# KAIST-VICLab/pronerf

Hardware: AMD Instinct MI355X
Metric: rays/sec (and ms/1008x756 frame) LLFF Fern 8-sample infer (higher is better)
Workload: dtype bf16 (NeRF MLP operands) + f16 (refine MLP operands); fp32 accumulate + f16 | f16x2 (sampler MLP: plain fp16 pass for every ray, split fp16 hi+lo operands = fp32-grade for the rays whose depth order that pass cannot decide; fp32 accumulate)

## Files before the change

include/pronerf_hip.h:

```cpp
#ifndef PRONERF_HIP_H
#define PRONERF_HIP_H

#include <stdint.h>

#ifdef __cplusplus
extern "C" {
#endif

#define PNRF_ABI_VERSION 1

#define PNRF_E_ARG (-1)
#define PNRF_E_SHAPE (-2)
#define PNRF_E_STATE (-3)

#define PNRF_NET_SAMPLER 0
#define PNRF_NET_REFINE 1
#define PNRF_NET_NERF 2
#define PNRF_NET_NERFCLS 3

typedef struct pnrf_mlp pnrf_mlp_t;
typedef struct pnrf_ctx pnrf_ctx_t;
typedef struct pnrf_trainer pnrf_trainer_t;
typedef struct pnrf_scene pnrf_scene_t;

// ... 54 lines not shown
                          float* refine_in, int64_t n, void* stream);
int pnrf_refine_input_train_fwd(const float* rays, const float* or_rays, const float* depth_sorted,
                                const float* img4, const float* poses, const float* K, const int64_t* ref_nos,
                                int nv, int nb, int Hf, int Wf, float eps, int layout, float* refine_in,
                                int64_t n, void* stream);
int pnrf_composite_fwd(const float* raw, const float* z, const float* rays_d, int d_stride,
                       const float* add, const float* mul, const float* noise, float clamp,
                       int white_bkgd, float* rgb, float* disp, float* acc, float* weights,
                       float* depth, int64_t n, int s, void* stream);

int pnrf_sampler_fwd(const pnrf_mlp_t* h, const float* rays, int64_t n, float* depth_sorted,
                     float* add_sorted, float* mul_sorted, int64_t* sort_idx, float* mm_rgb,
                     float* depth_raw, void* stream);
#define PNRF_SAMPLER_KAPPA 2.0f
int64_t pnrf_sampler_workspace_bytes(int64_t n);
int pnrf_sampler_fwd_ws(const pnrf_mlp_t* h, const float* rays, int64_t n, float* depth_sorted, float* add_sorted,
                        float* mul_sorted, int64_t* sort_idx, float* mm_rgb, float* depth_raw, void* workspace,
                        int64_t workspace_bytes, float kappa, void* stream);
int pnrf_refine_fwd(const pnrf_mlp_t* h, const float* refine_in, const float* rays,
                    const float* depth_sorted, float* z, float* pts, int64_t n, void* stream);
int pnrf_refine_project_fwd(const pnrf_mlp_t* h, const float* rays, const float* or_rays, const float* depth_sorted,
                            const float* img4, const float* proj, int nb, int Hf, int Wf, float eps, float* z,
                            float* pts, int64_t n, void* stream);
int pnrf_refine_train_fwd(const pnrf_mlp_t* h, const float* refine_in, const float* rays,
                          const float* depth_sorted, const float* jitter, int jitter_dir, float* z, float* pts,
                          float* rgb0, int64_t n, void* stream);
int pnrf_nerf_fwd(const pnrf_mlp_t* h, const float* pts, const float* rays, const float* z,
                  const float* add_sorted, const float* mul_sorted, float* rgbd, float* raw,
                  int64_t n, void* stream);

int pnrf_nerf_train_fwd(const pnrf_mlp_t* h, const float* pts, const float* rays, const float* z,
                        const float* add_sorted, const float* mul_sorted, const float* noise, float clamp,
                        int white_bkgd, int S, float* rgbd, float* raw, int64_t n, void* stream);
int pnrf_explore_fwd(const float* z8, const float* rays, const float* jitter, int n_mult, int dir1, int dir2,
                     float* z_out, float* pts_out, int64_t n, void* stream);

int pnrf_ctx_create(const pnrf_mlp_t* sampler, const pnrf_mlp_t* refine, const pnrf_mlp_t* nerf,
                    int64_t max_rays, pnrf_ctx_t** out);
int pnrf_ctx_free(pnrf_ctx_t* ctx);
int pnrf_render_rays_fwd(pnrf_ctx_t* ctx, const float* rays, const float* or_rays,
                         const float* img4, const float* proj, int nb, int Hf, int Wf, float eps,
                         float* rgbd, int64_t* sort_idx, int64_t n, void* stream);
int pnrf_ctx_set_sampler_kappa(pnrf_ctx_t* ctx, float kappa);
int pnrf_ctx_get_sampler_kappa(const pnrf_ctx_t* ctx, float* kappa);
int pnrf_ctx_sampler_stats(pnrf_ctx_t* ctx, int64_t* rays_second_pass);
int pnrf_ctx_sampler_saturated(pnrf_ctx_t* ctx, int64_t* rays_third_pass);
#define PNRF_NERF_SKIP_NEVER 0
#define PNRF_NERF_SKIP_AUTO 1
#define PNRF_NERF_SKIP_ALWAYS 2
#define PNRF_NERF_SKIP_MIN_RAYS 8192
#define PNRF_NERF_SKIP_DEAD_PERCENT 2
int pnrf_ctx_set_nerf_skip(pnrf_ctx_t* ctx, int mode);
int pnrf_ctx_nerf_live(pnrf_ctx_t* ctx, int64_t* live_columns, int* list_mode);
int pnrf_ctx_profile_begin(pnrf_ctx_t* ctx, int max_frames);
int pnrf_ctx_profile_end(pnrf_ctx_t* ctx, float* ms, int* frames);


int pnrf_composite_bwd(const float* raw, const float* z, const float* rays_d, int d_stride, const float* add,
                       const float* mul, const float* noise, float clamp, int white_bkgd, const float* d_rgb,
                       float* d_raw, float* d_z, float* d_add, float* d_mul, int64_t n, int s, void* stream);
int pnrf_composite_bwd_maps(const float* raw, const float* z, const float* rays_d, int d_stride, const float* add,
                            const float* mul, const float* noise, float clamp, int white_bkgd, const float* d_rgb,
                            const float* d_disp, const float* d_acc, const float* d_weights, const float* d_depth,
                            const float* d_z_in, float* d_raw, float* d_z, float* d_add, float* d_mul, int64_t n, int s,
                            void* stream);
int pnrf_posenc_bwd(const float* x, const float* d_out, float* d_x, int64_t n, int n_freq, void* stream);
// ... 134 lines not shown
```

pronerf_amd/_lib.py:

```python
from __future__ import annotations

import ctypes as C
import os

_HERE = os.path.dirname(os.path.abspath(__file__))
LIB_PATH = os.path.join(_HERE, 'lib', 'libpronerf_hip.so')

NET_SAMPLER, NET_REFINE, NET_NERF, NET_NERFCLS = 0, 1, 2, 3
VARIANTS = {'default': 0, 'sampler_f32': 1, 'sampler_f32_full': 2, 'bf16_32x32': 3, 'nerf_4x64': 4, 'sampler_split': 5, 'bf16': 6, 'f16': 7, 'refine_16x16': 8}
ABI_VERSION = 1


class PnrfError(RuntimeError):
    pass


_p = C.c_void_p
_i64 = C.c_int64
_f = C.c_float
_i = C.c_int

SIGNATURES = {
    'pnrf_abi_version': (_i, []),
    'pnrf_last_error': (C.c_char_p, []),
    'pnrf_mlp_pack': (_i, [_i, C.POINTER(_p), C.POINTER(_p), C.POINTER(_i), C.POINTER(_i), _i, C.POINTER(_p)]),
    'pnrf_mlp_pack_image': (_i, [_i, C.POINTER(_p), C.POINTER(_p), C.POINTER(_i), C.POINTER(_i), _i, _p, _i64, C.POINTER(_i64)]),
    'pnrf_mlp_repack': (_i, [_p, C.POINTER(_p), C.POINTER(_p), C.POINTER(_i), C.POINTER(_i), _i, _p]),
    'pnrf_mlp_free': (_i, [_p]),
    'pnrf_mlp_serialize': (_i, [_p, _p, _i64, C.POINTER(_i64)]),
    'pnrf_mlp_deserialize': (_i, [_p, _i64, C.POINTER(_p)]),
    'pnrf_mlp_kind': (_i, [_p, C.POINTER(_i), C.POINTER(_i), C.POINTER(_i), C.POINTER(_i)]),
    'pnrf_mlp_skips': (_i, [_p, C.POINTER(C.c_uint32)]),
    'pnrf_mlp_set_variant': (_i, [_p, _i]),
    'pnrf_mlp_set_shape': (_i, [_p, _i]),
    'pnrf_mlp_fwd': (_i, [_p, _p, _p, _p, _i64, _i, _p]),
    'pnrf_posenc_fwd': (_i, [_p, _p, _i64, _i, _p]),
    'pnrf_plucker_fwd': (_i, [_p, _p, _p, _i64, _p]),
    'pnrf_ray_encode_fwd': (_i, [_p, _p, _i64, _i, _p]),
    'pnrf_frame_rays_fwd': (_i, [C.POINTER(_f), C.POINTER(_f), _i, _i, _f, _f, _f, _f, _i64, _i64, _p, _p, _p]),
    'pnrf_frame_rays_blocks_fwd': (_i, [C.POINTER(_f), C.POINTER(_f), _i, _i, _f, _f, _f, _f, _i64, _i64, _i64, _i64, _p, _p, _p]),
    'pnrf_ndc_rays_fwd': (_i, [_p, _p, _i, _i, _f, _f, _p, _p, _i64, _p]),
    'pnrf_warp_trt_fwd': (_i, [_p, _p, _p, _p, _i64, _p, _p, _i, _i, _i, _i64, _p]),
    'pnrf_warp_train_fwd': (_i, [_p, _p, _p, _p, _i64, _p, _p, _p, _i, _i, _i, _i64, _p]),
    'pnrf_refine_input_train_fwd': (_i, [_p, _p, _p, _p, _p, _p, _p, _i, _i, _i, _i, _f, _i, _p, _i64, _p]),
    'pnrf_refine_train_fwd': (_i, [_p, _p, _p, _p, _p, _i, _p, _p, _p, _i64, _p]),
    'pnrf_nerf_train_fwd': (_i, [_p, _p, _p, _p, _p, _p, _p, _f, _i, _i, _p, _p, _i64, _p]),
    'pnrf_explore_fwd': (_i, [_p, _p, _p, _i, _i, _i, _p, _p, _i64, _p]),
    'pnrf_images_pack': (_i, [_p, _p, _i, _i, _i, _p]),
    'pnrf_refine_input_fwd': (_i, [_p, _p, _p, _p, _p, _i, _i, _i, _f, _p, _i64, _p]),
    'pnrf_composite_fwd': (_i, [_p, _p, _p, _i, _p, _p, _p, _f, _i, _p, _p, _p, _p, _p, _i64, _i, _p]),
    'pnrf_sampler_fwd': (_i, [_p, _p, _i64, _p, _p, _p, _p, _p, _p, _p]),
    'pnrf_sampler_workspace_bytes': (_i64, [_i64]),
    'pnrf_sampler_fwd_ws': (_i, [_p, _p, _i64, _p, _p, _p, _p, _p, _p, _p, _i64, _f, _p]),
    'pnrf_refine_fwd': (_i, [_p, _p, _p, _p, _p, _p, _i64, _p]),
    'pnrf_refine_project_fwd': (_i, [_p, _p, _p, _p, _p, _p, _i, _i, _i, _f, _p, _p, _i64, _p]),
    'pnrf_nerf_fwd': (_i, [_p, _p, _p, _p, _p, _p, _p, _p, _i64, _p]),
    'pnrf_ctx_create': (_i, [_p, _p, _p, _i64, C.POINTER(_p)]),
    'pnrf_ctx_free': (_i, [_p]),
    'pnrf_render_rays_fwd': (_i, [_p, _p, _p, _p, _p, _i, _i, _i, _f, _p, _p, _i64, _p]),
    'pnrf_ctx_sampler_stats': (_i, [_p, C.POINTER(_i64)]),
    'pnrf_ctx_set_sampler_kappa': (_i, [_p, _f]),
    'pnrf_ctx_get_sampler_kappa': (_i, [_p, C.POINTER(_f)]),
    'pnrf_ctx_sampler_saturated': (_i, [_p, C.POINTER(_i64)]),
    'pnrf_ctx_set_nerf_skip': (_i, [_p, _i]),
    'pnrf_ctx_nerf_live': (_i, [_p, C.POINTER(_i64), C.POINTER(_i)]),
    'pnrf_ctx_profile_begin': (_i, [_p, _i]),
    'pnrf_ctx_profile_end': (_i, [_p, C.POINTER(C.c_float), C.POINTER(_i)]),
    'pnrf_linspace': (_i, [_f, _f, _i, C.POINTER(_f)]),
    'pnrf_image_metrics_workspace_bytes': (_i64, [_i, _i, _i]),
    'pnrf_image_metrics_fwd': (_i, [_p, _i, _p, _i, _i, _i, C.POINTER(_f), _i, _f, _f, _f, _p, _p, _p, _i64, _p]),
    'pnrf_ssim_loss_workspace_bytes': (_i64, [_i, _i, _i, _i]),
    'pnrf_ssim_loss_fwd': (_i, [_p, _i, _i64, _p, _i, _i64, _i, _i, _i, C.POINTER(_f), _i, _f, _f, _f, _p, _p, _p, _i64, _p]),
    'pnrf_frame_to8b_fwd': (_i, [_p, _i, _p, _i, _i64, _p, _p, _p, _i64, _p]),
    'pnrf_png_segment_rows': (_i, []),
    'pnrf_png_max_bytes': (_i64, [_i, _i, _i]),
    'pnrf_png_workspace_bytes': (_i64, [_i, _i, _i]),
    'pnrf_png_encode_host': (_i, [_p, _i64, _i, _i, _i, _i, _p, _i64, C.POINTER(_i64)]),
    'pnrf_png_encode_fwd': (_i, [_p, _i64, _i, _i, _i, _i, _p, _i64, _p, _p, _i64, _p]),
    'pnrf_lpips_create': (_i, [C.c_char_p, C.POINTER(_p), C.POINTER(_p), C.POINTER(_i), _i, C.POINTER(_p), C.POINTER(_i), C.POINTER(_p)]),
    'pnrf_lpips_free': (_i, [_p]),
    'pnrf_lpips_tap_dims': (_i, [C.c_char_p, _i, _i, C.POINTER(_i)]),
    'pnrf_lpips_workspace_bytes': (_i64, [_p, _i, _i]),
    'pnrf_lpips_fwd': (_i, [_p, _p, _i, _p, _i, _i, _i, _i, _p, _p, _p, _i64, _p]),
    'pnrf_lpips_layer_workspace_bytes': (_i64, [_p, _i, _i, _i, _i]),
    'pnrf_lpips_layer_fwd': (_i, [_p, _i, _i, _p, _i, _i, _p, _p, _i64, _p]),
    'pnrf_lpips_loss_workspace_bytes': (_i64, [_p, _i, _i, _i]),
    'pnrf_lpips_loss_fwd': (_i, [_p, _p, _i, _i64, _p, _i, _i64, _i, _i, _i, _i, _p, _p, _p, _i64, _p]),
    'pnrf_lpips_layer_bwd_workspace_bytes': (_i64, [_p, _i, _i, _i, _i, _i]),
    'pnrf_lpips_layer_bwd': (_i, [_p, _i, _i, _i, _i, _p, _i, _i, _p, _p, _p, _p, _i64, _p]),
# ... 89 lines not shown
```

pronerf_amd/csrc/pnrf_mlp_kernels.hip:

```cpp
#include <type_traits>

#include "pnrf_common.h"
#include "pnrf_geom.h"

#ifndef PNRF_LAST_TMAX
#define PNRF_LAST_TMAX 1
#endif
#ifndef PNRF_OLD_PRIO
#define PNRF_OLD_PRIO 0
#endif
#ifndef PNRF_YOUNG_PRIO
#define PNRF_YOUNG_PRIO 1
#endif

using namespace pnrf;

namespace {



template <int N, int I = 0, class F>
__device__ __forceinline__ void static_for(F&& f) {
  if constexpr (I < N) {
    f(std::integral_constant<int, I>{});
// ... 1675 lines not shown
  }
  return make_float4(s0, s1, s2, s3);
}

typedef __bf16 bf16x2_t __attribute__((ext_vector_type(2)));
__device__ __forceinline__ int relu_pack_bf16(float a, float b) {
#ifdef PNRF_RELU_F32
  return __builtin_bit_cast(int, bf16x2_t{(__bf16)act_fast(a, ACT_RELU), (__bf16)act_fast(b, ACT_RELU)});
#else
  int pk;
  asm("v_cvt_pk_bf16_f32 %0, %1, %2" : "=v"(pk) : "v"(a), "v"(b));
  return __builtin_bit_cast(int, __builtin_elementwise_max(__builtin_bit_cast(i16x2_t, pk), i16x2_t{0, 0}));
#endif
}
template <class P>
__device__ __forceinline__ int relu_pack(float a, float b) {
  if constexpr (std::is_same<P, PrecBf16>::value) return relu_pack_bf16(a, b);
  return __builtin_bit_cast(int, __builtin_elementwise_max(__builtin_bit_cast(i16x2_t, P::cvt_pk(a, b)), i16x2_t{0, 0}));
}
template <int NCB, class P = PrecBf16>
struct HiddenEpi16 {
  typename P::v8 (&Bn)[NCB][NB_KS_H];
  __device__ __forceinline__ void operator()(int tp, int pc, f32x4 (&acc)[2][NCB], int cb0) const {
#pragma unroll
    for (int cb = cb0; cb < cb0 + 2; ++cb) {
      i32x4_t w = __builtin_bit_cast(i32x4_t, Bn[cb][tp]);
      w[2 * pc] = relu_pack<P>(acc[pc][cb][0], acc[pc][cb][1]);
      w[2 * pc + 1] = relu_pack<P>(acc[pc][cb][2], acc[pc][cb][3]);
      Bn[cb][tp] = __builtin_bit_cast(typename P::v8, w);
    }
  }
};

template <bool CLS, int NCB, class P, int NW, bool LIST>
__device__ __forceinline__ void nerf16_body(const NerfArgs& a) {
  constexpr int TPB = 64 * NW;
  using Epi = HiddenEpi16<NCB, P>;
  using v8 = typename P::v8;
  if (a.skip && a.skip[SKIP_MODE] != (LIST ? SKIP_MODE_LIST : SKIP_MODE_DENSE)) return;
  const int nlive = LIST ? a.skip[SKIP_LIVE] : 0;
  const int nbatch = LIST ? (nlive + NW * 16 * NCB - 1) / (NW * 16 * NCB) : a.nbatch;
  if constexpr (LIST) {
    if ((int)blockIdx.x >= nbatch) {
      if (threadIdx.x == 0 && atomicAdd(a.queue + 1, 1) == (int)gridDim.x - 1) { a.queue[0] = 0; a.queue[1] = 0; }
      return;
    }
  }
  P::enter();
  extern __shared__ __attribute__((aligned(16))) char smem[];
  float* bias_lds = (float*)(smem + RING_BYTES);
  WStream<NW> st;
  st.init(a.blob, a.nslots, smem);
  st.prologue();
  for (int i = threadIdx.x; i < a.nbias; i += TPB) bias_lds[i] = a.bias[i];
  __syncthreads();
  const int lane = threadIdx.x & 63, wave = threadIdx.x >> 6, c16 = lane & 15, g = lane >> 4;
  int pe_c[4];
  float pe_sc[4];
#pragma unroll
  for (int j4 = 0; j4 < 4; ++j4) {
    const int q = 4 * g + j4;
    pe_c[j4] = q % 3;
    pe_sc[j4] = (float)(1 << (2 * (q / 3)));
  }
  const float pe_vs = (float)(1 << g);
  const int64_t nrows = a.n * a.S;
  own_the_simd<NW>();
  young_half_priority<NW>();
  const char* ringlane = smem + lane * 16;
  const float* biaslane = bias_lds + 4 * g;
  const bool composite = !LIST && a.S == 8 && a.rgbd;

  __shared__ __attribute__((aligned(16))) int s_next[4];
  for (int batch = blockIdx.x; batch < nbatch;) {
    int q_pend = 0;
    if (a.queue && threadIdx.x == 0) q_pend = atomicAdd(a.queue, 1);
    int64_t row[NCB];
    bool valid[NCB];
    v8 Bo[NCB][NB_KS_H], Bn[NCB][NB_KS_H], Bx[NCB];
    float e_dn[NCB], e_z[NCB], e_add[NCB], e_mul[NCB], e_noise[NCB];
    static_for<NCB>([&](auto cbc) {
      constexpr int cb = decltype(cbc)::value;
      row[cb] = (int64_t)batch * (NW * 16 * NCB) + wave * (16 * NCB) + cb * 16 + c16;
      valid[cb] = row[cb] < (LIST ? (int64_t)nlive : nrows);
      int64_t rr = valid[cb] ? row[cb] : nrows - 1;
      if constexpr (LIST) {
        rr = a.list[valid[cb] ? row[cb] : (int64_t)nlive - 1];
        row[cb] = rr;
      }
      const float* pp = a.pts + rr * 3;
      const float* ry = a.rays + (a.S == 8 ? (rr >> 3) : rr / a.S) * 11;
      const float x3[3] = {pp[0], pp[1], pp[2]};
      const float v3[3] = {ry[8], ry[9], ry[10]};
      if (composite) {
        e_dn[cb] = ray_dir_norm(ry);
        e_z[cb] = a.z[rr]; e_add[cb] = a.add ? a.add[rr] : 0.f; e_mul[cb] = a.mul ? a.mul[rr] : 1.f;
        e_noise[cb] = a.noise ? a.noise[rr] : 0.f;
      }
      float f0[16], fx[8];
#pragma unroll
      for (int j4 = 0; j4 < 4; ++j4) {
        const float xv = pe_c[j4] == 0 ? x3[0] : (pe_c[j4] == 1 ? x3[1] : x3[2]);
        float s, co;
        pe_sincos_scaled(xv, pe_sc[j4], s, co);
        f0[4 * j4 + 0] = s; f0[4 * j4 + 1] = co;
        f0[4 * j4 + 2] = 2.f * s * co; f0[4 * j4 + 3] = (co - s) * (co + s);
      }
      if (g == 3) { f0[12] = x3[0]; f0[13] = x3[1]; f0[14] = x3[2]; f0[15] = 0.f; }
#pragma unroll
      for (int c = 0; c < 3; ++c) pe_sincos_scaled(v3[c], pe_vs, fx[2 * c], fx[2 * c + 1]);
      fx[6] = g == 0 ? v3[0] : (g == 1 ? v3[2] : 0.f);
      fx[7] = g == 0 ? v3[1] : 0.f;
#pragma unroll
      for (int ks = 0; ks < NB_KS0; ++ks) {
        float v[8];
#pragma unroll
        for (int j = 0; j < 8; ++j) v[j] = f0[ks * 8 + j];
        Bo[cb][ks] = P::pack(v);
      }
      Bx[cb] = P::pack(fx);
    });
    f32x4 fin[2][NCB], pend[2][NCB];
    if constexpr (!CLS) {
      auto hidden = [&](v8(&in)[NCB][NB_KS_H], v8(&out)[NCB][NB_KS_H], int l) {
        f32x4 np[2][NCB];
        layer_b16<NB_KS_H, NB_NTP_H, NB_POS_H, NCB, v8>(st, ringlane, biaslane + (1 + l) * W_HID, [&](int cb, int ks) { return in[cb][ks]; }, Epi{out},
                                               [&](int pc, int cb0) { Epi{in}(NB_NTP_H - 1, pc, pend, cb0); }, np);
#pragma unroll
        for (int t = 0; t < 2; ++t)
#pragma unroll
          for (int cb = 0; cb < NCB; ++cb) pend[t][cb] = np[t][cb];
      };
      layer_b16<NB_KS0, NB_NTP_H, 0, NCB, v8>(st, ringlane, biaslane, [&](int cb, int ks) { return Bo[cb][ks < NB_KS0 ? ks : 0]; }, Epi{Bn}, [](int, int) {}, pend);
      const int nhid = PNRF_NHID(a.nhid, N_NHID);
      auto last_layer = [&](v8(&in)[NCB][NB_KS_H]) {
        layer_b16<NB_KS_LAST, 1, NB_POS_LAST, NCB, v8, PNRF_LAST_TMAX>(
            st, ringlane, biaslane + (1 + nhid) * W_HID, [&](int cb, int ks) { return ks < NB_KS_H ? in[cb][ks < NB_KS_H ? ks : 0] : Bx[cb]; },
            [&](int, int, f32x4(&)[2][NCB], int) {}, [&](int pc, int cb0) { Epi{in}(NB_NTP_H - 1, pc, pend, cb0); }, fin);
      };
      bool in_bo = false;
      for (int l = 0; l < nhid; l += 2) {
        hidden(Bn, Bo, l);
        if (l + 1 >= nhid) { in_bo = true; break; }
        hidden(Bo, Bn, l + 1);
      }
      if (in_bo) last_layer(Bo);
      else last_layer(Bn);
#pragma unroll
      for (int i = 0; i < NB_SLOTS_PAD; ++i) st.begin();
    } else {
      v8 Pz[NCB][NB_KS0];
#pragma unroll
      for (int cb = 0; cb < NCB; ++cb)
#pragma unroll
        for (int k = 0; k < NB_KS0; ++k) Pz[cb][k] = Bo[cb][k];
      auto hidden = [&](v8(&in)[NCB][NB_KS_H], v8(&out)[NCB][NB_KS_H], int l, auto posc) {
        constexpr int POS = decltype(posc)::value;
        f32x4 np[2][NCB];
        layer_b16<NB_KS_H, NB_NTP_H, POS, NCB, v8>(st, ringlane, biaslane + l * W_HID, [&](int cb, int ks) { return in[cb][ks]; }, Epi{out},
                                          [&](int pc, int cb0) { Epi{in}(NB_NTP_H - 1, pc, pend, cb0); }, np);
#pragma unroll
        for (int t = 0; t < 2; ++t)
#pragma unroll
          for (int cb = 0; cb < NCB; ++cb) pend[t][cb] = np[t][cb];
      };
      layer_b16<NB_KS0, NB_NTP_H, 0, NCB, v8>(st, ringlane, biaslane, [&](int cb, int ks) { return Bo[cb][ks < NB_KS0 ? ks : 0]; }, Epi{Bn}, [](int, int) {}, pend);
      for (int l = 1; l < 5; l += 2) {
        hidden(Bn, Bo, l, std::integral_constant<int, CB_POS_E1>{});
        hidden(Bo, Bn, l + 1, std::integral_constant<int, CB_POS_E1>{});
      }
      {
        f32x4 np[2][NCB];
        layer_b16<CB_KS5, NB_NTP_H, CB_POS_E5, NCB, v8>(
            st, ringlane, biaslane + 5 * W_HID,
            [&](int cb, int ks) { return ks < NB_KS_H ? Bn[cb][ks < NB_KS_H ? ks : 0] : Pz[cb][ks >= NB_KS_H ? ks - NB_KS_H : 0]; }, Epi{Bo},
            [&](int pc, int cb0) { Epi{Bn}(NB_NTP_H - 1, pc, pend, cb0); }, np);
#pragma unroll
        for (int t = 0; t < 2; ++t)
#pragma unroll
          for (int cb = 0; cb < NCB; ++cb) pend[t][cb] = np[t][cb];
      }
      hidden(Bo, Bn, 6, std::integral_constant<int, CB_POS_E6>{});
      hidden(Bn, Bo, 7, std::integral_constant<int, CB_POS_E6>{});
      f32x4 al[2][NCB];
      layer_b16<NB_KS_LAST, CB_NTP89, CB_POS_E89, NCB, v8>(
          st, ringlane, biaslane + CB_BIAS_E89, [&](int cb, int ks) { return ks < NB_KS_H ? Bo[cb][ks < NB_KS_H ? ks : 0] : Bx[cb]; }, Epi{Bn},
          [&](int pc, int cb0) { Epi{Bo}(NB_NTP_H - 1, pc, pend, cb0); }, al);
      layer_b16<CB_KS10, 1, CB_POS_E10, NCB, v8, PNRF_LAST_TMAX>(st, ringlane, biaslane + CB_BIAS_E10, [&](int cb, int ks) { return Bn[cb][ks < CB_KS10 ? ks : 0]; },
                                        [&](int, int, f32x4(&)[2][NCB], int) {}, [](int, int) {}, fin);
#pragma unroll
      for (int cb = 0; cb < NCB; ++cb) fin[0][cb][3] = al[0][cb][0];
#pragma unroll
      for (int i = 0; i < CB_SLOTS_PAD; ++i) st.begin();
    }

    static_for<NCB>([&](auto cbc) {
      constexpr int cb = decltype(cbc)::value;
      const int64_t rr = valid[cb] ? row[cb] : nrows - 1;
      float r0 = fin[0][cb][0], r1 = fin[0][cb][1], r2 = fin[0][cb][2], r3 = fin[0][cb][3];
      if (a.raw && valid[cb] && g == 0) *(float4*)(a.raw + row[cb] * 4) = make_float4(r0, r1, r2, r3);
      if (!composite) return;
      const int64_t ray = rr >> 3;
      const int s = (int)(rr & 7);
      const float4 px = composite8_dpp(a, r0, r1, r2, r3, e_dn[cb], e_z[cb], e_add[cb], e_mul[cb], e_noise[cb], s);
      const float s0 = px.x, s1 = px.y, s2 = px.z, s3 = px.w;
      if (valid[cb] && g == 0 && s == 0) *(float4*)(a.rgbd + ray * 4) = make_float4(s0, s1, s2, s3);
    });
    if (a.queue) {
      if (threadIdx.x == 0) s_next[0] = (int)gridDim.x + q_pend;
      __syncthreads();
      batch = s_next[0];
    } else {
      batch += gridDim.x;
    }
  }
  st.drain();
  if (a.queue && threadIdx.x == 0) {
    if (atomicAdd(a.queue + 1, 1) == (int)gridDim.x - 1) { a.queue[0] = 0; a.queue[1] = 0; }
  }
}

template <bool CLS, int NCB = 2, class P = PrecBf16, int NW = 16 / NCB>
__global__ __launch_bounds__(64 * NW, NCB == 2 ? 2 : 1) void nerf16_kernel(NerfArgs a) {
  nerf16_body<CLS, NCB, P, NW, false>(a);
}
template <bool CLS, int NCB = 2, class P = PrecBf16, int NW = 16 / NCB>
__global__ __launch_bounds__(64 * NW, NCB == 2 ? 2 : 1) void nerf16_list_kernel(NerfArgs a) {
  nerf16_body<CLS, NCB, P, NW, true>(a);
}

constexpr int LIVE_TILES = 8;
__global__ __launch_bounds__(256) void nerf_live_list_kernel(const float* __restrict__ mul, int64_t ncols, int* __restrict__ list, int* skip, int force, int dead_percent) {
  __shared__ int s_cnt[4], s_base;
  const int lane = threadIdx.x & 63, wave = threadIdx.x >> 6;
  int64_t c0[LIVE_TILES];
  float4 m[LIVE_TILES];
#pragma unroll
  for (int t = 0; t < LIVE_TILES; ++t) {
    c0[t] = (((int64_t)blockIdx.x * LIVE_TILES + t) * 256 + threadIdx.x) * 4;
    m[t] = make_float4(0.f, 0.f, 0.f, 0.f);
    if (c0[t] < ncols) m[t] = *(const float4*)(mul + c0[t]);
  }
  int place[LIVE_TILES][4], total = 0;
#pragma unroll
  for (int t = 0; t < LIVE_TILES; ++t) {
    const float mv[4] = {m[t].x, m[t].y, m[t].z, m[t].w};
#pragma unroll
    for (int j = 0; j < 4; ++j) {
      const unsigned long long b = __ballot(mv[j] > 0.f);
      place[t][j] = total + (int)__builtin_amdgcn_mbcnt_hi((unsigned)(b >> 32), __builtin_amdgcn_mbcnt_lo((unsigned)b, 0u));
      total += __popcll(b);
    }
  }
  if (lane == 0) s_cnt[wave] = total;
  __syncthreads();
  if (threadIdx.x == 0) {
    const int mine = s_cnt[0] + s_cnt[1] + s_cnt[2] + s_cnt[3];
    const unsigned long long old = atomicAdd((unsigned long long*)(skip + SKIP_RUN), (1ull << 32) | (unsigned long long)(unsigned)mine);
    s_base = (int)(unsigned)old;
    if ((int)(old >> 32) == (int)gridDim.x - 1) {
      const int64_t live = (int64_t)(unsigned)old + mine;
      skip[SKIP_LIVE] = (int)live;
      skip[SKIP_MODE] = (force || (ncols - live) * 100 >= (int64_t)dead_percent * ncols) ? SKIP_MODE_LIST : SKIP_MODE_DENSE;
      skip[SKIP_RUN] = 0; skip[SKIP_DONE] = 0;
    }
  }
  __syncthreads();
  int base = s_base;
  for (int w = 0; w < wave; ++w) base += s_cnt[w];
#pragma unroll
  for (int t = 0; t < LIVE_TILES; ++t) {
    const float mv[4] = {m[t].x, m[t].y, m[t].z, m[t].w};
#pragma unroll
    for (int j = 0; j < 4; ++j)
      if (mv[j] > 0.f) list[base + place[t][j]] = (int)(c0[t] + j);
  }
}

__global__ __launch_bounds__(256) void nerf_composite_kernel(NerfArgs a) {
  if (a.skip[SKIP_MODE] != SKIP_MODE_LIST) return;
  const int64_t ncols = a.n * 8;
  const int64_t col = (int64_t)blockIdx.x * 256 + threadIdx.x;
  const bool valid = col < ncols;
  const int64_t rr = valid ? col : ncols - 1;
  const float* ry = a.rays + (rr >> 3) * 11;
  const float dn = ray_dir_norm(ry);
  const float zc = a.z[rr], ad = a.add[rr], mu = a.mul[rr];
  float4 r = make_float4(0.f, 0.f, 0.f, 0.f);
  if (mu > 0.f) r = *(const float4*)(a.raw + rr * 4);
  const int s = (int)(rr & 7);
  const float4 px = composite8_dpp(a, r.x, r.y, r.z, r.w, dn, zc, ad, mu, 0.f, s);
  if (valid && s == 0) *(float4*)(a.rgbd + (rr >> 3) * 4) = px;
}

int g_num_cu = 0;
int num_cu() {
  if (!g_num_cu) {
    int dev = 0;
    hipDeviceProp_t p;
    if (hipGetDevice(&dev) == hipSuccess && hipGetDeviceProperties(&p, dev) == hipSuccess) g_num_cu = p.multiProcessorCount;
    if (g_num_cu <= 0) g_num_cu = 256;
  }
  return g_num_cu;
}

template <class K, class A>
int launch_mlp(K kern, const A& a, int tpb, size_t lds, int nbatch, hipStream_t stream) {
  {
    hipError_t e = hipFuncSetAttribute((const void*)kern, hipFuncAttributeMaxDynamicSharedMemorySize, (int)((lds + 8191) & ~(size_t)4095));
    if (e != hipSuccess) {
      set_error("hipFuncSetAttribute(max dynamic LDS) failed: %s", hipGetErrorString(e));
      return (int)e;
    }
  }
  const int ncu = num_cu();
  const int grid = nbatch < ncu ? nbatch : ncu;
  hipLaunchKernelGGL(kern, dim3(grid), dim3(tpb), lds, stream, a);
  hipError_t e = hipGetLastError();
  if (e != hipSuccess) {
    set_error("kernel launch failed: %s", hipGetErrorString(e));
    return (int)e;
  }
// ... 240 lines not shown
extern "C" int pnrf_refine_project_fwd(const pnrf_mlp_t* h, const float* rays, const float* or_rays, const float* depth_sorted, const float* img4,
                                       const float* proj, int nb, int Hf, int Wf, float eps, float* z, float* pts, int64_t n, void* stream) {
  PNRF_REQUIRE(h && h->net == PNRF_NET_REFINE, PNRF_E_ARG, "pnrf_refine_project_fwd: handle is not a refine net");
  PNRF_REQUIRE(n >= 0 && nb == h->nb && Hf >= 2 && Wf >= 2 && (int64_t)Hf * Wf * nb < (int64_t)1 << 27, PNRF_E_ARG,
               "pnrf_refine_project_fwd: bad sizes (nb must be the refine net's num_neighbor = %d, got %d; nb * Hf * Wf must stay below 2^27 texels)", h->nb, nb);
  if (n == 0) return 0;
  PNRF_REQUIRE(rays && or_rays && depth_sorted && img4 && proj && z && pts, PNRF_E_ARG, "pnrf_refine_project_fwd: null pointer");

  RefineArgs a = {};
  a.blob = h->d_blob; a.bias = h->d_bias; a.nslots = h->nslots; a.nbias = h->nbias;
  a.n = n;
  a.or_rays = or_rays; a.img4 = (const float4*)img4; a.proj = proj; a.Hf = Hf; a.Wf = Wf; a.eps = eps;
  a.rays = rays; a.depth_sorted = depth_sorted; a.z = z; a.pts = pts;
  return refine_launch<1, 1>(h, a, n, (hipStream_t)stream);
}

extern "C" int pnrf_nerf_fwd(const pnrf_mlp_t* h, const float* pts, const float* rays, const float* z,
                             const float* add_sorted, const float* mul_sorted, float* rgbd, float* raw,
                             int64_t n, void* stream) {
  PNRF_REQUIRE(n == 0 || (z && add_sorted && mul_sorted && rgbd), PNRF_E_ARG, "pnrf_nerf_fwd: null pointer");
  return pnrf_nerf_train_fwd(h, pts, rays, z, add_sorted, mul_sorted, nullptr, 0.f, 0, 8, rgbd, raw, n, stream);
}

extern "C" int pnrf_nerf_train_fwd(const pnrf_mlp_t* h, const float* pts, const float* rays, const float* z,
                                   const float* add_sorted, const float* mul_sorted, const float* noise, float clampv, int white_bkgd,
                                   int S, float* rgbd, float* raw, int64_t n, void* stream) {
  return pnrf_nerf_fwd_queue_impl(h, pts, rays, z, add_sorted, mul_sorted, noise, clampv, white_bkgd, S, rgbd, raw, n, nullptr, stream);
}

int pnrf_nerf_fwd_queue_impl(const pnrf_mlp_t* h, const float* pts, const float* rays, const float* z,
                             const float* add_sorted, const float* mul_sorted, const float* noise, float clampv, int white_bkgd,
                             int S, float* rgbd, float* raw, int64_t n, int* queue, void* stream) {
  return pnrf_nerf_fwd_skip_impl(h, pts, rays, z, add_sorted, mul_sorted, noise, clampv, white_bkgd, S, rgbd, raw, n, queue, nullptr, nullptr, 0, stream);
}

bool pnrf_nerf_skip_supported(const pnrf_mlp_t* h) { return h && (h->variant == PNRF_VARIANT_DEFAULT || h->variant == PNRF_VARIANT_F16); }

int pnrf_nerf_fwd_skip_impl(const pnrf_mlp_t* h, const float* pts, const float* rays, const float* z,
                            const float* add_sorted, const float* mul_sorted, const float* noise, float clampv, int white_bkgd,
                            int S, float* rgbd, float* raw, int64_t n, int* queue, int* skip, int* list, int force_list, void* stream) {
  PNRF_REQUIRE(h && (h->net == PNRF_NET_NERF || h->net == PNRF_NET_NERFCLS), PNRF_E_ARG, "pnrf_nerf_fwd: handle is not a nerf net");
  PNRF_REQUIRE(n >= 0 && S >= 1 && (n == 0 || (pts && rays)), PNRF_E_ARG, "pnrf_nerf_fwd: null pointer / negative n / bad S");
  PNRF_REQUIRE(n == 0 || (S == 8 ? ((rgbd && z) || raw) : (raw && !rgbd)), PNRF_E_ARG,
               "pnrf_nerf_train_fwd: S == 8 needs rgbd (+z) or raw; S != 8 writes raw only (composite with pnrf_composite_fwd)");
  PNRF_REQUIRE((add_sorted == nullptr) == (mul_sorted == nullptr), PNRF_E_ARG, "pnrf_nerf_train_fwd: add and mul go together");
  PNRF_REQUIRE(!skip || (pnrf_nerf_skip_supported(h) && S == 8 && rgbd && z && mul_sorted && raw && list && queue && !noise && clampv == 0.f && !white_bkgd &&
                         n * 8 < ((int64_t)1 << 31)),
               PNRF_E_ARG, "pnrf_nerf_fwd: the compacted-column path needs the default engine, S == 8, rgbd, z, add / mul, a queue and its workspace");
  if (n == 0) return 0;
  NerfArgs a = {};
  a.blob = h->d_blob; a.bias = h->d_bias; a.nslots = h->nslots; a.nbias = h->nbias;
  a.n = n;
  a.pts = pts; a.rays = rays; a.z = z; a.add = add_sorted; a.mul = mul_sorted; a.rgbd = rgbd; a.raw = skip ? nullptr : raw;
  a.noise = noise; a.white_bkgd = white_bkgd; a.clampv = clampv; a.S = S; a.nhid = h->nhid;
  a.queue = h->variant == PNRF_VARIANT_BF16_32X32 ? nullptr : queue;
  a.skip = skip;
  const size_t lds = RING_BYTES + (size_t)h->nbias * 4;
  const int rows = 256;
  a.nbatch = (int)((n * S + rows - 1) / rows);
  const bool b16 = h->variant != PNRF_VARIANT_BF16_32X32;
  const bool f16 = h->variant == PNRF_VARIANT_F16;
  if (b16) {
    a.blob = f16 ? h->d_blob_f16 : h->d_blob_b16; a.nslots = f16 ? h->nslots_f16 : h->nslots_b16; a.bias = h->d_bias_b16; a.nbias = h->nbias_b16;
  }
  const size_t lds16 = RING_BYTES + (size_t)h->nbias_b16 * 4;
  hipStream_t st = (hipStream_t)stream;
  const bool narrow = b16 && h->variant != PNRF_VARIANT_NERF_4X64 && stage_shape(h, n * S, 32) == SHAPE_NARROW;
  if (narrow) a.nbatch = (int)((n * S + 127) / 128);
  if (skip) {
    const int64_t ncols = n * 8;
    hipLaunchKernelGGL(nerf_live_list_kernel, dim3((unsigned)((ncols + 1024 * LIVE_TILES - 1) / (1024 * LIVE_TILES))), dim3(256), 0, st, mul_sorted, ncols, list, skip, force_list,
                       PNRF_NERF_SKIP_DEAD_PERCENT);
    PNRF_LAUNCH_CHECK();
  }
  const bool cls = h->net == PNRF_NET_NERFCLS;
  auto fused = [&](bool list_mode) -> int {
    NerfArgs b = a;
    if (list_mode) { b.list = list; b.raw = raw; b.rgbd = nullptr; }
#define PNRF_NERF16(CLS_, P_, NW_, TPB_, LDS_)                                                                                \
    (list_mode ? launch_mlp(nerf16_list_kernel<CLS_, 2, P_, NW_>, b, TPB_, LDS_, b.nbatch, st) : launch_mlp(nerf16_kernel<CLS_, 2, P_, NW_>, b, TPB_, LDS_, b.nbatch, st))
    if (cls) {
      if (narrow) return f16 ? PNRF_NERF16(true, PrecF16, 4, 256, narrow_lds(lds16)) : PNRF_NERF16(true, PrecBf16, 4, 256, narrow_lds(lds16));
      if (f16) return PNRF_NERF16(true, PrecF16, 8, 512, lds16);
      if (h->variant == PNRF_VARIANT_NERF_4X64) return launch_mlp(nerf16_kernel<true, 4>, b, 256, lds16, b.nbatch, st);
      if (b16) return PNRF_NERF16(true, PrecBf16, 8, 512, lds16);
      return launch_mlp(nerf_kernel<1, 8, true, true>, b, 512, lds, b.nbatch, st);
    }
    if (narrow) return f16 ? PNRF_NERF16(false, PrecF16, 4, 256, narrow_lds(lds16)) : PNRF_NERF16(false, PrecBf16, 4, 256, narrow_lds(lds16));
    if (f16) return PNRF_NERF16(false, PrecF16, 8, 512, lds16);
    if (h->variant == PNRF_VARIANT_NERF_4X64) return launch_mlp(nerf16_kernel<false, 4>, b, 256, lds16, b.nbatch, st);
    if (b16) return PNRF_NERF16(false, PrecBf16, 8, 512, lds16);
#undef PNRF_NERF16
    PNRF_REQUIRE(h->nhid == N_NHID, PNRF_E_SHAPE, "PNRF_VARIANT_BF16_32X32 is built for netdepth %d; this net has netdepth %d — the default engine takes any", N_NHID + 2, h->nhid + 2);
    return launch_mlp(nerf_kernel<1, 8, true, false>, b, 512, lds, b.nbatch, st);
  };
  if (int rc = fused(false)) return rc;
  if (!skip) return 0;
  if (int rc = fused(true)) return rc;
  NerfArgs c = a;
  c.raw = raw;
  hipLaunchKernelGGL(nerf_composite_kernel, dim3((unsigned)((n * 8 + 255) / 256)), dim3(256), 0, st, c);
  PNRF_LAUNCH_CHECK();
  return 0;
}

extern "C" int pnrf_mlp_fwd(const pnrf_mlp_t* h, const float* x, const float* x_views, float* y, int64_t m, int head_act, void* stream) {
  PNRF_REQUIRE(h, PNRF_E_ARG, "pnrf_mlp_fwd: null handle");
  PNRF_REQUIRE(m >= 0 && (m == 0 || (x && y)), PNRF_E_ARG, "pnrf_mlp_fwd: null pointer / negative m");
  PNRF_REQUIRE((h->net != PNRF_NET_NERF && h->net != PNRF_NET_NERFCLS) || m == 0 || x_views, PNRF_E_ARG, "pnrf_mlp_fwd: the nerf nets need x_views [m,27]");
  if (m == 0) return 0;
  const size_t lds = RING_BYTES + (size_t)h->nbias * 4;
  if (h->net == PNRF_NET_SAMPLER) {
    SamplerArgs a = {};
    PNRF_REQUIRE(!h->skips, PNRF_E_SHAPE, "pnrf_mlp_fwd: the module-level sampler forward (unfolded first layer) is not built for nets with skip connections (mmnetskips); "
                 "the fused operators (pnrf_sampler_fwd / pnrf_render_rays_fwd) take them");
    PNRF_REQUIRE(h->npts == S_NPTS && h->d_blob, PNRF_E_SHAPE, "pnrf_mlp_fwd: the module-level sampler forward (unfolded first layer) is built for N_point_ray_enc = %d, "
                 "this sampler has %d; the fused operators (pnrf_sampler_fwd / pnrf_render_rays_fwd) take any", S_NPTS, h->npts);
    a.blob = h->d_blob; a.bias = h->d_bias; a.nslots = h->nslots; a.nbias = h->nbias; a.nhid = h->nhid;
    a.n = m; a.nbatch = (int)((m + 127) / 128);
    a.x = x; a.in0 = h->d_in0; a.y = y; a.outmap = h->d_out; a.head_act = head_act;
    return launch_mlp(sampler_kernel<0>, a, 512, lds, a.nbatch, (hipStream_t)stream);
  }
  if (h->net == PNRF_NET_REFINE) {
    RefineArgs a = {};
    a.blob = h->d_blob; a.bias = h->d_bias; a.nslots = h->nslots; a.nbias = h->nbias;
    a.n = m; a.nbatch = (int)((m + 127) / 128);
    a.x = x; a.y = y; a.outmap = h->d_out; a.head_act = head_act; a.nhid = h->nhid; a.nb = h->nb;
    const bool bf16 = h->variant == PNRF_VARIANT_BF16;
    if (!bf16) { a.blob = h->d_blob_f16; a.nslots = h->nslots_f16; }
    auto go = [&](auto nvc) {
      constexpr int NV = decltype(nvc)::value;
// ... 22 lines not shown
```

pronerf_amd/ops.py:

```python
from __future__ import annotations

import ctypes as C

import numpy as np
import torch

from . import _lib
from ._lib import NET_NERF, NET_NERFCLS, NET_REFINE, NET_SAMPLER, PnrfError, check

f32 = torch.float32


def _ptr(t):
    return C.c_void_p(0) if t is None else C.c_void_p(t.data_ptr())


def _stream():
    return C.c_void_p(torch.cuda.current_stream().cuda_stream)


def _chk(t, name, shape_tail=None):
    if not isinstance(t, torch.Tensor) or not t.is_cuda:
        raise PnrfError(f'{name}: expected a GPU tensor (pronerf_amd has no CPU path)')
    if t.dtype != f32:
# ... 337 lines not shown
    check(_lib.load().pnrf_sampler_fwd(mlp.handle, _ptr(rays), n, _ptr(depth), _ptr(add), _ptr(mul), _ptr(idx), _ptr(rgb), _ptr(draw), _stream()),
          'pnrf_sampler_fwd')
    return depth, idx, add, mul, rgb, draw


def refine_fwd(mlp: PackedMLP, refine_in, rays, depth_sorted):
    refine_in = _chk(refine_in, 'refine_in', (mlp.in_dim,)); rays = _chk(rays, 'rays', (11,)); depth_sorted = _chk(depth_sorted, 'depth_sorted', (8,))
    n, dev = rays.shape[0], rays.device
    z = torch.empty(n, 8, device=dev, dtype=f32); pts = torch.empty(n, 8, 3, device=dev, dtype=f32)
    check(_lib.load().pnrf_refine_fwd(mlp.handle, _ptr(refine_in), _ptr(rays), _ptr(depth_sorted), _ptr(z), _ptr(pts), n, _stream()), 'pnrf_refine_fwd')
    return z, pts


def refine_project_fwd(mlp: PackedMLP, rays, or_rays, depth_sorted, img4, proj, eps=1e-5):
    rays = _chk(rays, 'rays', (11,)); or_rays = _chk(or_rays, 'or_rays', (11,)); depth_sorted = _chk(depth_sorted, 'depth_sorted', (8,))
    img4 = _chk(img4, 'img4', (4,)); proj = _chk(proj, 'proj', (3, 4))
    nb, Hf, Wf, _ = img4.shape
    if proj.shape[0] != nb:
        raise PnrfError(f'refine_project_fwd: {nb} packed images but {proj.shape[0]} projection matrices')
    n, dev = rays.shape[0], rays.device
    z = torch.empty(n, 8, device=dev, dtype=f32); pts = torch.empty(n, 8, 3, device=dev, dtype=f32)
    check(_lib.load().pnrf_refine_project_fwd(mlp.handle, _ptr(rays), _ptr(or_rays), _ptr(depth_sorted), _ptr(img4), _ptr(proj), nb, Hf, Wf, eps,
                                              _ptr(z), _ptr(pts), n, _stream()), 'pnrf_refine_project_fwd')
    return z, pts


def nerf_fwd(mlp: PackedMLP, pts, rays, z, add, mul, want_raw=False):
    pts = _chk(pts, 'pts', (8, 3)); rays = _chk(rays, 'rays', (11,)); z = _chk(z, 'z', (8,)); add = _chk(add, 'add', (8,)); mul = _chk(mul, 'mul', (8,))
    n, dev = rays.shape[0], rays.device
    rgbd = torch.empty(n, 4, device=dev, dtype=f32)
    raw = torch.empty(n, 8, 4, device=dev, dtype=f32) if want_raw else None
    check(_lib.load().pnrf_nerf_fwd(mlp.handle, _ptr(pts), _ptr(rays), _ptr(z), _ptr(add), _ptr(mul), _ptr(rgbd), _ptr(raw), n, _stream()), 'pnrf_nerf_fwd')
    return rgbd, raw


class RenderContext:

    def __init__(self, sampler: PackedMLP, refine: PackedMLP, nerf: PackedMLP, max_rays: int):
        self._keep = (sampler, refine, nerf)
        h = C.c_void_p()
        check(_lib.load().pnrf_ctx_create(sampler.handle, refine.handle, nerf.handle, int(max_rays), C.byref(h)), 'pnrf_ctx_create')
        self.handle = h
        self.max_rays = int(max_rays)

    def __del__(self):
        try:
            if getattr(self, 'handle', None):
                _lib.load().pnrf_ctx_free(self.handle)
                self.handle = None
        except Exception:
            pass

    STAGES = ('sampler_kernel', 'refine_kernel', 'nerf_kernel')

    def sampler_stats(self):
        v = C.c_int64()
        check(_lib.load().pnrf_ctx_sampler_stats(self.handle, C.byref(v)), 'pnrf_ctx_sampler_stats')
        return int(v.value)

    def sampler_saturated(self):
        v = C.c_int64()
        check(_lib.load().pnrf_ctx_sampler_saturated(self.handle, C.byref(v)), 'pnrf_ctx_sampler_saturated')
        return int(v.value)

    def set_sampler_kappa(self, kappa):
        check(_lib.load().pnrf_ctx_set_sampler_kappa(self.handle, float(kappa)), 'pnrf_ctx_set_sampler_kappa')
# ... 925 lines not shown
```

Baseline: 182.2 million.

## Unify nerf dense and live-list paths into one column kernel launch

The nerf MLP kernel's list mode becomes a 'cols' mode that reads the skip mode at runtime. It walks either the compacted live-column list or every column, so the skip path no longer needs both a dense launch and a list launch. The composite kernel now also handles the dense case, reading raw for all columns. An optional prefetch of the next batch's list ids (off by default) and a new pnrf_nerf_cols_fwd API with its Python workspace wrapper are added. The cost is that dense-mode skip paths now go through raw-to-global plus a separate composite pass instead of the in-kernel fused composite.

```diff
diff --git a/include/pronerf_hip.h b/include/pronerf_hip.h
--- a/include/pronerf_hip.h
+++ b/include/pronerf_hip.h
@@ -110,6 +110,9 @@
 int pnrf_nerf_train_fwd(const pnrf_mlp_t* h, const float* pts, const float* rays, const float* z,
                         const float* add_sorted, const float* mul_sorted, const float* noise, float clamp,
                         int white_bkgd, int S, float* rgbd, float* raw, int64_t n, void* stream);
+int pnrf_nerf_cols_fwd(const pnrf_mlp_t* h, const float* pts, const float* rays, const float* z,
+                       const float* add_sorted, const float* mul_sorted, float* rgbd, float* raw_ws, int* list_ws,
+                       int* state, int64_t n, int force_list, void* stream);
 int pnrf_explore_fwd(const float* z8, const float* rays, const float* jitter, int n_mult, int dir1, int dir2,
                      float* z_out, float* pts_out, int64_t n, void* stream);
 
diff --git a/pronerf_amd/_lib.py b/pronerf_amd/_lib.py
--- a/pronerf_amd/_lib.py
+++ b/pronerf_amd/_lib.py
@@ -55,6 +55,7 @@
     'pnrf_refine_fwd': (_i, [_p, _p, _p, _p, _p, _p, _i64, _p]),
     'pnrf_refine_project_fwd': (_i, [_p, _p, _p, _p, _p, _p, _i, _i, _i, _f, _p, _p, _i64, _p]),
     'pnrf_nerf_fwd': (_i, [_p, _p, _p, _p, _p, _p, _p, _p, _i64, _p]),
+    'pnrf_nerf_cols_fwd': (_i, [_p, _p, _p, _p, _p, _p, _p, _p, _p, _p, _i64, _i, _p]),
     'pnrf_ctx_create': (_i, [_p, _p, _p, _i64, C.POINTER(_p)]),
     'pnrf_ctx_free': (_i, [_p]),
     'pnrf_render_rays_fwd': (_i, [_p, _p, _p, _p, _p, _i, _i, _i, _f, _p, _p, _i64, _p]),
diff --git a/pronerf_amd/csrc/pnrf_mlp_kernels.hip b/pronerf_amd/csrc/pnrf_mlp_kernels.hip
--- a/pronerf_amd/csrc/pnrf_mlp_kernels.hip
+++ b/pronerf_amd/csrc/pnrf_mlp_kernels.hip
@@ -1731,15 +1731,24 @@
   }
 };
 
-template <bool CLS, int NCB, class P, int NW, bool LIST>
+#ifndef PNRF_NERF_IDS_AHEAD
+#define PNRF_NERF_IDS_AHEAD 0
+#endif
+template <bool CLS, int NCB, class P, int NW, bool COLS>
 __device__ __forceinline__ void nerf16_body(const NerfArgs& a) {
   constexpr int TPB = 64 * NW;
   using Epi = HiddenEpi16<NCB, P>;
   using v8 = typename P::v8;
-  if (a.skip && a.skip[SKIP_MODE] != (LIST ? SKIP_MODE_LIST : SKIP_MODE_DENSE)) return;
-  const int nlive = LIST ? a.skip[SKIP_LIVE] : 0;
-  const int nbatch = LIST ? (nlive + NW * 16 * NCB - 1) / (NW * 16 * NCB) : a.nbatch;
-  if constexpr (LIST) {
+  if (!COLS && a.skip && a.skip[SKIP_MODE] != SKIP_MODE_DENSE) return;
+  const bool by_list = COLS && __builtin_amdgcn_readfirstlane(a.skip[SKIP_MODE]) == SKIP_MODE_LIST;
+  const int nlive = COLS ? (by_list ? __builtin_amdgcn_readfirstlane(a.skip[SKIP_LIVE]) : (int)(a.n * a.S)) : 0;
+#ifdef PNRF_DIAG_NERF_NOHOP
+  const bool hop = false;
+#else
+  const bool hop = by_list;
+#endif
+  const int nbatch = COLS ? (nlive + NW * 16 * NCB - 1) / (NW * 16 * NCB) : a.nbatch;
+  if constexpr (COLS) {
     if ((int)blockIdx.x >= nbatch) {
       if (threadIdx.x == 0 && atomicAdd(a.queue + 1, 1) == (int)gridDim.x - 1) { a.queue[0] = 0; a.queue[1] = 0; }
       return;
@@ -1768,9 +1777,14 @@
   young_half_priority<NW>();
   const char* ringlane = smem + lane * 16;
   const float* biaslane = bias_lds + 4 * g;
-  const bool composite = !LIST && a.S == 8 && a.rgbd;
+  const bool composite = !COLS && a.S == 8 && a.rgbd;
 
   __shared__ __attribute__((aligned(16))) int s_next[4];
+  constexpr bool AHEAD = COLS && PNRF_NERF_IDS_AHEAD;
+  int ids_next[NCB];
+  bool have_next = false;
+#pragma unroll
+  for (int cb = 0; cb < NCB; ++cb) ids_next[cb] = 0;
   for (int batch = blockIdx.x; batch < nbatch;) {
     int q_pend = 0;
     if (a.queue && threadIdx.x == 0) q_pend = atomicAdd(a.queue, 1);
@@ -1778,14 +1792,34 @@
     bool valid[NCB];
     v8 Bo[NCB][NB_KS_H], Bn[NCB][NB_KS_H], Bx[NCB];
     float e_dn[NCB], e_z[NCB], e_add[NCB], e_mul[NCB], e_noise[NCB];
+    int ids[NCB];
+    if constexpr (COLS) {
+#pragma unroll
+      for (int cb = 0; cb < NCB; ++cb) {
+        const int c = batch * (NW * 16 * NCB) + wave * (16 * NCB) + cb * 16 + c16;
+        valid[cb] = c < nlive;
+        ids[cb] = valid[cb] ? c : nlive - 1;
+      }
+      if (hop) {
+        if (AHEAD && have_next) {
+#pragma unroll
+          for (int cb = 0; cb < NCB; ++cb) ids[cb] = ids_next[cb];
+        } else {
+#pragma unroll
+          for (int cb = 0; cb < NCB; ++cb) ids[cb] = a.list[ids[cb]];
+        }
+      }
+    }
     static_for<NCB>([&](auto cbc) {
       constexpr int cb = decltype(cbc)::value;
-      row[cb] = (int64_t)batch * (NW * 16 * NCB) + wave * (16 * NCB) + cb * 16 + c16;
-      valid[cb] = row[cb] < (LIST ? (int64_t)nlive : nrows);
-      int64_t rr = valid[cb] ? row[cb] : nrows - 1;
-      if constexpr (LIST) {
-        rr = a.list[valid[cb] ? row[cb] : (int64_t)nlive - 1];
+      int64_t rr;
+      if constexpr (COLS) {
+        rr = ids[cb];
         row[cb] = rr;
+      } else {
+        row[cb] = (int64_t)batch * (NW * 16 * NCB) + wave * (16 * NCB) + cb * 16 + c16;
+        valid[cb] = row[cb] < nrows;
+        rr = valid[cb] ? row[cb] : nrows - 1;
       }
       const float* pp = a.pts + rr * 3;
       const float* ry = a.rays + (a.S == 8 ? (rr >> 3) : rr / a.S) * 11;
@@ -1820,6 +1854,32 @@
       Bx[cb] = P::pack(fx);
     });
     f32x4 fin[2][NCB], pend[2][NCB];
+    if constexpr (AHEAD) {
+      if (hop && a.queue && threadIdx.x == 0) s_next[1] = (int)gridDim.x + q_pend;
+    }
+    auto ids_ahead = [&]() {
+      if constexpr (AHEAD) {
+        have_next = false;
+        if (hop) {
+          const int nb = a.queue ? __builtin_amdgcn_readfirstlane(s_next[1]) : batch + (int)gridDim.x;
+          have_next = nb < nbatch;
+          if (have_next) {
+#pragma unroll
+            for (int cb = 0; cb < NCB; ++cb) {
+              const int c = nb * (NW * 16 * NCB) + wave * (16 * NCB) + cb * 16 + c16;
+              asm volatile("global_load_dword %0, %1, off" : "=v"(ids_next[cb]) : "v"(a.list + (c < nlive ? c : nlive - 1)) : "memory");
+            }
+          }
+        }
+      }
+    };
+    auto ids_landed = [&]() {
+      if constexpr (AHEAD) {
+        asm volatile("s_waitcnt vmcnt(%0)" ::"n"(WStream<NW>::LOADS_PER_WAVE * PD) : "memory");
+#pragma unroll
+        for (int cb = 0; cb < NCB; ++cb) asm volatile("" : "+v"(ids_next[cb]));
+      }
+    };
     if constexpr (!CLS) {
       auto hidden = [&](v8(&in)[NCB][NB_KS_H], v8(&out)[NCB][NB_KS_H], int l) {
         f32x4 np[2][NCB];
@@ -1831,6 +1891,7 @@
           for (int cb = 0; cb < NCB; ++cb) pend[t][cb] = np[t][cb];
       };
       layer_b16<NB_KS0, NB_NTP_H, 0, NCB, v8>(st, ringlane, biaslane, [&](int cb, int ks) { return Bo[cb][ks < NB_KS0 ? ks : 0]; }, Epi{Bn}, [](int, int) {}, pend);
+      ids_ahead();
       const int nhid = PNRF_NHID(a.nhid, N_NHID);
       auto last_layer = [&](v8(&in)[NCB][NB_KS_H]) {
         layer_b16<NB_KS_LAST, 1, NB_POS_LAST, NCB, v8, PNRF_LAST_TMAX>(
@@ -1847,6 +1908,7 @@
       else last_layer(Bn);
 #pragma unroll
       for (int i = 0; i < NB_SLOTS_PAD; ++i) st.begin();
+      ids_landed();
     } else {
       v8 Pz[NCB][NB_KS0];
 #pragma unroll
@@ -1864,6 +1926,7 @@
           for (int cb = 0; cb < NCB; ++cb) pend[t][cb] = np[t][cb];
       };
       layer_b16<NB_KS0, NB_NTP_H, 0, NCB, v8>(st, ringlane, biaslane, [&](int cb, int ks) { return Bo[cb][ks < NB_KS0 ? ks : 0]; }, Epi{Bn}, [](int, int) {}, pend);
+      ids_ahead();
       for (int l = 1; l < 5; l += 2) {
         hidden(Bn, Bo, l, std::integral_constant<int, CB_POS_E1>{});
         hidden(Bo, Bn, l + 1, std::integral_constant<int, CB_POS_E1>{});
@@ -1891,6 +1954,7 @@
       for (int cb = 0; cb < NCB; ++cb) fin[0][cb][3] = al[0][cb][0];
 #pragma unroll
       for (int i = 0; i < CB_SLOTS_PAD; ++i) st.begin();
+      ids_landed();
     }
 
     static_for<NCB>([&](auto cbc) {
@@ -1924,7 +1988,7 @@
   nerf16_body<CLS, NCB, P, NW, false>(a);
 }
 template <bool CLS, int NCB = 2, class P = PrecBf16, int NW = 16 / NCB>
-__global__ __launch_bounds__(64 * NW, NCB == 2 ? 2 : 1) void nerf16_list_kernel(NerfArgs a) {
+__global__ __launch_bounds__(64 * NW, NCB == 2 ? 2 : 1) void nerf16_cols_kernel(NerfArgs a) {
   nerf16_body<CLS, NCB, P, NW, true>(a);
 }
 
@@ -1940,6 +2004,11 @@
     m[t] = make_float4(0.f, 0.f, 0.f, 0.f);
     if (c0[t] < ncols) m[t] = *(const float4*)(mul + c0[t]);
   }
+#ifdef PNRF_DIAG_NERF_ALL_LIVE
+#pragma unroll
+  for (int t = 0; t < LIVE_TILES; ++t)
+    if (c0[t] < ncols) m[t] = make_float4(1.f, 1.f, 1.f, 1.f);
+#endif
   int place[LIVE_TILES][4], total = 0;
 #pragma unroll
   for (int t = 0; t < LIVE_TILES; ++t) {
@@ -1977,7 +2046,7 @@
 }
 
 __global__ __launch_bounds__(256) void nerf_composite_kernel(NerfArgs a) {
-  if (a.skip[SKIP_MODE] != SKIP_MODE_LIST) return;
+  const bool all = a.skip[SKIP_MODE] != SKIP_MODE_LIST;
   const int64_t ncols = a.n * 8;
   const int64_t col = (int64_t)blockIdx.x * 256 + threadIdx.x;
   const bool valid = col < ncols;
@@ -1986,7 +2055,7 @@
   const float dn = ray_dir_norm(ry);
   const float zc = a.z[rr], ad = a.add[rr], mu = a.mul[rr];
   float4 r = make_float4(0.f, 0.f, 0.f, 0.f);
-  if (mu > 0.f) r = *(const float4*)(a.raw + rr * 4);
+  if (all || mu > 0.f) r = *(const float4*)(a.raw + rr * 4);
   const int s = (int)(rr & 7);
   const float4 px = composite8_dpp(a, r.x, r.y, r.z, r.w, dn, zc, ad, mu, 0.f, s);
   if (valid && s == 0) *(float4*)(a.rgbd + (rr >> 3) * 4) = px;
@@ -2293,6 +2362,15 @@
                              const float* add_sorted, const float* mul_sorted, const float* noise, float clampv, int white_bkgd,
                              int S, float* rgbd, float* raw, int64_t n, int* queue, void* stream) {
   return pnrf_nerf_fwd_skip_impl(h, pts, rays, z, add_sorted, mul_sorted, noise, clampv, white_bkgd, S, rgbd, raw, n, queue, nullptr, nullptr, 0, stream);
+}
+
+extern "C" int pnrf_nerf_cols_fwd(const pnrf_mlp_t* h, const float* pts, const float* rays, const float* z,
+                                  const float* add_sorted, const float* mul_sorted, float* rgbd, float* raw_ws, int* list_ws,
+                                  int* state, int64_t n, int force_list, void* stream) {
+  PNRF_REQUIRE(h && pnrf_nerf_skip_supported(h), PNRF_E_ARG, "pnrf_nerf_cols_fwd: needs a nerf handle on the default engine (or PNRF_VARIANT_F16)");
+  PNRF_REQUIRE(n == 0 || (pts && rays && z && add_sorted && mul_sorted && rgbd && raw_ws && list_ws && state), PNRF_E_ARG, "pnrf_nerf_cols_fwd: null pointer");
+  PNRF_REQUIRE(((uintptr_t)state & 7) == 0, PNRF_E_ARG, "pnrf_nerf_cols_fwd: state must be 8-byte aligned");
+  return pnrf_nerf_fwd_skip_impl(h, pts, rays, z, add_sorted, mul_sorted, nullptr, 0.f, 0, 8, rgbd, raw_ws, n, state, state + 2, list_ws, force_list != 0, stream);
 }
 
 bool pnrf_nerf_skip_supported(const pnrf_mlp_t* h) { return h && (h->variant == PNRF_VARIANT_DEFAULT || h->variant == PNRF_VARIANT_F16); }
@@ -2335,11 +2413,11 @@
     PNRF_LAUNCH_CHECK();
   }
   const bool cls = h->net == PNRF_NET_NERFCLS;
-  auto fused = [&](bool list_mode) -> int {
+  auto fused = [&](bool cols) -> int {
     NerfArgs b = a;
-    if (list_mode) { b.list = list; b.raw = raw; b.rgbd = nullptr; }
+    if (cols) { b.list = list; b.raw = raw; b.rgbd = nullptr; }
 #define PNRF_NERF16(CLS_, P_, NW_, TPB_, LDS_)                                                                                \
-    (list_mode ? launch_mlp(nerf16_list_kernel<CLS_, 2, P_, NW_>, b, TPB_, LDS_, b.nbatch, st) : launch_mlp(nerf16_kernel<CLS_, 2, P_, NW_>, b, TPB_, LDS_, b.nbatch, st))
+    (cols ? launch_mlp(nerf16_cols_kernel<CLS_, 2, P_, NW_>, b, TPB_, LDS_, b.nbatch, st) : launch_mlp(nerf16_kernel<CLS_, 2, P_, NW_>, b, TPB_, LDS_, b.nbatch, st))
     if (cls) {
       if (narrow) return f16 ? PNRF_NERF16(true, PrecF16, 4, 256, narrow_lds(lds16)) : PNRF_NERF16(true, PrecBf16, 4, 256, narrow_lds(lds16));
       if (f16) return PNRF_NERF16(true, PrecF16, 8, 512, lds16);
@@ -2355,9 +2433,8 @@
     PNRF_REQUIRE(h->nhid == N_NHID, PNRF_E_SHAPE, "PNRF_VARIANT_BF16_32X32 is built for netdepth %d; this net has netdepth %d — the default engine takes any", N_NHID + 2, h->nhid + 2);
     return launch_mlp(nerf_kernel<1, 8, true, false>, b, 512, lds, b.nbatch, st);
   };
-  if (int rc = fused(false)) return rc;
+  if (int rc = fused(skip != nullptr)) return rc;
   if (!skip) return 0;
-  if (int rc = fused(true)) return rc;
   NerfArgs c = a;
   c.raw = raw;
   hipLaunchKernelGGL(nerf_composite_kernel, dim3((unsigned)((n * 8 + 255) / 256)), dim3(256), 0, st, c);
diff --git a/pronerf_amd/ops.py b/pronerf_amd/ops.py
--- a/pronerf_amd/ops.py
+++ b/pronerf_amd/ops.py
@@ -393,6 +393,26 @@
     raw = torch.empty(n, 8, 4, device=dev, dtype=f32) if want_raw else None
     check(_lib.load().pnrf_nerf_fwd(mlp.handle, _ptr(pts), _ptr(rays), _ptr(z), _ptr(add), _ptr(mul), _ptr(rgbd), _ptr(raw), n, _stream()), 'pnrf_nerf_fwd')
     return rgbd, raw
+
+
+class NerfColsWorkspace:
+
+    def __init__(self, max_rays, device):
+        self.max_rays = int(max_rays)
+        self.raw = torch.zeros(self.max_rays, 8, 4, device=device, dtype=f32)
+        self.list = torch.zeros(self.max_rays * 8, device=device, dtype=torch.int32)
+        self.state = torch.zeros(6, device=device, dtype=torch.int32)
+
+
+def nerf_cols_fwd(mlp: PackedMLP, pts, rays, z, add, mul, ws: NerfColsWorkspace, force_list=False):
+    pts = _chk(pts, 'pts', (8, 3)); rays = _chk(rays, 'rays', (11,)); z = _chk(z, 'z', (8,)); add = _chk(add, 'add', (8,)); mul = _chk(mul, 'mul', (8,))
+    n, dev = rays.shape[0], rays.device
+    if n > ws.max_rays:
+        raise PnrfError(f'nerf_cols_fwd: {n} rays, the workspace holds {ws.max_rays}')
+    rgbd = torch.empty(n, 4, device=dev, dtype=f32)
+    check(_lib.load().pnrf_nerf_cols_fwd(mlp.handle, _ptr(pts), _ptr(rays), _ptr(z), _ptr(add), _ptr(mul), _ptr(rgbd), _ptr(ws.raw), _ptr(ws.list), _ptr(ws.state),
+                                         n, int(bool(force_list)), _stream()), 'pnrf_nerf_cols_fwd')
+    return rgbd
 
 
 class RenderContext:
```

New measurement: 182.7 million, median of 5. No clear change (+0.3%).
